# hamaadshah/gan_deeplearning4j

Hardware: AMD Instinct MI355X
Metric: images/sec (whole node) DCGAN 64x64 bf16 (higher is better)
Workload: dtype bf16; 1 GPU; model=dcgan64, global_batch=16384, z_size=128, parallelism=dp1

## Files before the change

gan_deeplearning4j_amd/ops/hip/gemm.hip:

```cpp

#include "conv_gather.h"

constexpr int TN_BM = 128, TN_BN = 128, TN_BK = 64;
constexpr int TN_TILE_B = TN_BM * TN_BK * 2;

DEV_INLINE bf16x8 tn_frag(const char* lds, int row, int kslot) {
  int byte = row * 128 + ((kslot ^ (row & 7)) * 16);
  return *(const bf16x8*)(lds + byte);
}

template <bool GATHER_A>
__global__ __launch_bounds__(256, 2) void gemm_tn_core(
    const unsigned short* __restrict__ A, const unsigned short* __restrict__ B,
    unsigned short* __restrict__ C, float* __restrict__ Cf,
    const float* __restrict__ bias, int M, int N, int K, long lda, long ldb,
    int act, float slope, ConvGather ga,
    const unsigned short* __restrict__ zp,
    float* __restrict__ bn_part) {
  __shared__ __attribute__((aligned(128))) char lds[4 * TN_TILE_B];
  auto abuf = [&](int i) -> char* { return lds + (i ? 2 * TN_TILE_B : 0); };
  auto bbuf = [&](int i) -> char* {
    return lds + TN_TILE_B + (i ? 2 * TN_TILE_B : 0);
  };

  const int nwgx = gridDim.x;
  const int bidx = xcd_remap(blockIdx.x, nwgx);
  const int m0 = bidx * TN_BM;
  const int n0 = blockIdx.y * TN_BN;

  const int wid = threadIdx.x >> 6;
  const int lane = threadIdx.x & 63;
  const int wr = wid >> 1, wc = wid & 1;
  const int fr = lane & 15, fq = lane >> 4;

  f32x4 acc[4][4];
  #pragma unroll
  for (int i = 0; i < 4; ++i)
    #pragma unroll
    for (int j = 0; j < 4; ++j) acc[i][j] = {0.f, 0.f, 0.f, 0.f};

  const int ntiles = K / TN_BK;
  TnGatherStager<256, unsigned short> gs;
  if (GATHER_A) {
    gs.init(ga, m0, M);
    gs.stage(A, ga, zp, 0, abuf(0));
  } else {
    tn_stage_rows<256, 4>(A, m0, M, lda, 0, abuf(0));
  }
  tn_stage_rows<256, 4>(B, n0, N, ldb, 0, bbuf(0));
  asm volatile("s_waitcnt vmcnt(0)" ::: "memory");
  __syncthreads();

  for (int t = 0; t < ntiles; ++t) {
    int cur = t & 1;
    if (t + 1 < ntiles) {
      if (GATHER_A)
        gs.stage(A, ga, zp, (t + 1) * TN_BK, abuf(cur ^ 1));
      else
        tn_stage_rows<256, 4>(A, m0, M, lda, (t + 1) * TN_BK, abuf(cur ^ 1));
      tn_stage_rows<256, 4>(B, n0, N, ldb, (t + 1) * TN_BK, bbuf(cur ^ 1));
    }
    const char* Al = abuf(cur);
    const char* Bl = bbuf(cur);
    #pragma unroll
    for (int kc = 0; kc < 2; ++kc) {
      bf16x8 a[4], b[4];
      #pragma unroll
      for (int mi = 0; mi < 4; ++mi)
        a[mi] = tn_frag(Al, wr * 64 + mi * 16 + fr, kc * 4 + fq);
      #pragma unroll
      for (int ni = 0; ni < 4; ++ni)
        b[ni] = tn_frag(Bl, wc * 64 + ni * 16 + fr, kc * 4 + fq);
      #pragma unroll
      for (int mi = 0; mi < 4; ++mi)
        #pragma unroll
        for (int ni = 0; ni < 4; ++ni)
          acc[mi][ni] = __builtin_amdgcn_mfma_f32_16x16x32_bf16(
              a[mi], b[ni], acc[mi][ni], 0, 0, 0);
    }
    asm volatile("s_waitcnt vmcnt(0)" ::: "memory");
    __syncthreads();
  }

  if (C != nullptr && (N & 7) == 0) {
    unsigned short* ctile = (unsigned short*)lds;
    __syncthreads();
    #pragma unroll
    for (int mi = 0; mi < 4; ++mi) {
      #pragma unroll
      for (int ni = 0; ni < 4; ++ni) {
        int lc = wc * 64 + ni * 16 + fr;
        float bv = bias != nullptr ? bias[min(n0 + lc, N - 1)] : 0.f;
        #pragma unroll
        for (int r = 0; r < 4; ++r) {
          int lr = wr * 64 + mi * 16 + fq * 4 + r;
          ctile[lr * 128 + lc] = f2bf(act_fwd(acc[mi][ni][r] + bv, act,
                                              slope));
        }
      }
    }
    __syncthreads();
    const int t = threadIdx.x;
    #pragma unroll
    for (int i = 0; i < 8; ++i) {
      int piece = i * 256 + t;
      int row = piece >> 4;
      int seg = piece & 15;
      int grow = m0 + row;
      int gcol = n0 + seg * 8;
      if (grow < M && gcol < N) {
        long crow = grow;
        if (GATHER_A && ga.mode == 2) crow = scatter_row(ga, grow);
        s16x8 v = *(const s16x8*)(ctile + row * 128 + seg * 8);
        if (gcol + 8 <= N) {
          *(s16x8*)(&C[crow * N + gcol]) = v;
        } else {
          for (int j = 0; j < 8 && gcol + j < N; ++j)
            C[crow * N + gcol + j] = (unsigned short)v[j];
        }
      }
    }
    if (bn_part != nullptr) {
      float* red = (float*)(lds + 2 * TN_TILE_B);
      const int col = t & 127;
      const int rl = t >> 7;
      float s = 0.f, ss = 0.f;
      for (int row = rl; row < 128; row += 2) {
        if (m0 + row < M) {
          float v = bf2f(ctile[row * 128 + col]);
          s += v;
          ss += v * v;
        }
      }
      red[t] = s;
      red[256 + t] = ss;
      __syncthreads();
      if (rl == 0 && n0 + col < N) {
        s += red[128 + col];
        ss += red[256 + 128 + col];
        bn_part[(long)blockIdx.x * 2 * N + n0 + col] = s;
        bn_part[(long)blockIdx.x * 2 * N + N + n0 + col] = ss;
      }
    }
    return;
  }
  #pragma unroll
  for (int mi = 0; mi < 4; ++mi) {
    #pragma unroll
    for (int ni = 0; ni < 4; ++ni) {
      int col = n0 + wc * 64 + ni * 16 + fr;
      if (col >= N) continue;
      float bv = bias != nullptr ? bias[col] : 0.f;
      #pragma unroll
      for (int r = 0; r < 4; ++r) {
        int row = m0 + wr * 64 + mi * 16 + fq * 4 + r;
        if (row >= M) continue;
        long crow = row;
        if (GATHER_A && ga.mode == 2) crow = scatter_row(ga, row);
        float v = act_fwd(acc[mi][ni][r] + bv, act, slope);
        if (C != nullptr)
          C[crow * N + col] = f2bf(v);
        else
          Cf[crow * N + col] = v;
      }
    }
  }
}

template <int KT, bool GATHER_A = false>
__global__ __launch_bounds__(256, 2) void gemm_tn_kshort(
    const unsigned short* __restrict__ A, const unsigned short* __restrict__ B,
    unsigned short* __restrict__ C, const float* __restrict__ bias, int M,
    int N, long lda, long ldb, int act, float slope, int direct_epi,
    ConvGather ga, const unsigned short* __restrict__ zp) {
  constexpr int NT = KT / TN_BK;
  __shared__ __attribute__((aligned(128))) char lds[2 * NT * TN_TILE_B];
  auto abuf = [&](int t) -> char* { return lds + t * TN_TILE_B; };
  auto bbuf = [&](int t) -> char* { return lds + (NT + t) * TN_TILE_B; };

  const int nwgx = gridDim.x;
  const int bidx = xcd_remap(blockIdx.x, nwgx);
  const int m0 = bidx * TN_BM;
  const int n0 = blockIdx.y * TN_BN;
  const int wid = threadIdx.x >> 6;
  const int lane = threadIdx.x & 63;
  const int wr = wid >> 1, wc = wid & 1;
  const int fr = lane & 15, fq = lane >> 4;

  f32x4 acc[4][4];
  #pragma unroll
  for (int i = 0; i < 4; ++i)
    #pragma unroll
    for (int j = 0; j < 4; ++j) acc[i][j] = {0.f, 0.f, 0.f, 0.f};

  TnGatherStager<256, unsigned short> gs;
  if (GATHER_A) gs.init(ga, m0, M);
  #pragma unroll
  for (int t = 0; t < NT; ++t) {
    if (GATHER_A)
      gs.stage(A, ga, zp, t * TN_BK, abuf(t));
    else
      tn_stage_rows<256, 4>(A, m0, M, lda, t * TN_BK, abuf(t));
    tn_stage_rows<256, 4>(B, n0, N, ldb, t * TN_BK, bbuf(t));
  }
  asm volatile("s_waitcnt vmcnt(0)" ::: "memory");
  __syncthreads();

  #pragma unroll
  for (int t = 0; t < NT; ++t) {
    const char* Al = abuf(t);
    const char* Bl = bbuf(t);
    #pragma unroll
    for (int kc = 0; kc < 2; ++kc) {
      bf16x8 a[4], b[4];
      #pragma unroll
      for (int mi = 0; mi < 4; ++mi)
        a[mi] = tn_frag(Al, wr * 64 + mi * 16 + fr, kc * 4 + fq);
      #pragma unroll
      for (int ni = 0; ni < 4; ++ni)
        b[ni] = tn_frag(Bl, wc * 64 + ni * 16 + fr, kc * 4 + fq);
      #pragma unroll
      for (int mi = 0; mi < 4; ++mi)
        #pragma unroll
        for (int ni = 0; ni < 4; ++ni)
          acc[mi][ni] = __builtin_amdgcn_mfma_f32_16x16x32_bf16(
              a[mi], b[ni], acc[mi][ni], 0, 0, 0);
    }
  }

  if ((N & 7) == 0 && direct_epi != 1) {
    unsigned short* ctile = (unsigned short*)lds;
    __syncthreads();
    #pragma unroll
    for (int mi = 0; mi < 4; ++mi) {
      #pragma unroll
      for (int ni = 0; ni < 4; ++ni) {
        int lc = wc * 64 + ni * 16 + fr;
        float bv = bias != nullptr ? bias[min(n0 + lc, N - 1)] : 0.f;
        #pragma unroll
        for (int r = 0; r < 4; ++r) {
          int lr = wr * 64 + mi * 16 + fq * 4 + r;
          ctile[lr * 128 + lc] = f2bf(act_fwd(acc[mi][ni][r] + bv, act,
                                              slope));
        }
      }
    }
    __syncthreads();
    const int t = threadIdx.x;
    #pragma unroll
    for (int i = 0; i < 8; ++i) {
      int piece = i * 256 + t;
      int row = piece >> 4;
      int seg = piece & 15;
      int grow = m0 + row;
      int gcol = n0 + seg * 8;
      if (grow < M && gcol + 8 <= N) {
        long crow = grow;
        if (GATHER_A && ga.mode == 2) crow = scatter_row(ga, grow);
        s16x8 v = *(const s16x8*)(ctile + row * 128 + seg * 8);
        if (direct_epi == 2)
          __builtin_nontemporal_store(v, (s16x8*)(&C[crow * N + gcol]));
        else
          *(s16x8*)(&C[crow * N + gcol]) = v;
      }
    }
    return;
  }
  #pragma unroll
  for (int mi = 0; mi < 4; ++mi)
    #pragma unroll
    for (int ni = 0; ni < 4; ++ni) {
      int col = n0 + wc * 64 + ni * 16 + fr;
      if (col >= N) continue;
      float bv = bias != nullptr ? bias[col] : 0.f;
      #pragma unroll
      for (int r = 0; r < 4; ++r) {
        int row = m0 + wr * 64 + mi * 16 + fq * 4 + r;
        if (row >= M) continue;
        long crow = row;
        if (GATHER_A && ga.mode == 2) crow = scatter_row(ga, row);
        C[crow * N + col] = f2bf(act_fwd(acc[mi][ni][r] + bv, act,
                                              slope));
      }
    }
}

constexpr int T2_BM = 256, T2_BN = 128, T2_BK = 64;
constexpr int T2_AT = T2_BM * T2_BK * 2;
constexpr int T2_BT = T2_BN * T2_BK * 2;

template <bool GATHER_A>
__global__ __launch_bounds__(512, 1) void gemm_tn_core256(
    const unsigned short* __restrict__ A, const unsigned short* __restrict__ B,
    unsigned short* __restrict__ C, const float* __restrict__ bias, int M,
    int N, int K, long lda, long ldb, int act, float slope, ConvGather ga,
    const unsigned short* __restrict__ zp) {
  extern __shared__ __attribute__((aligned(128))) char lds[];
  auto abuf = [&](int i) -> char* { return lds + (i ? T2_AT : 0); };
  auto bbuf = [&](int i) -> char* {
    return lds + 2 * T2_AT + (i ? T2_BT : 0);
  };

  const int nwgx = gridDim.x;
  const int bidx = xcd_remap(blockIdx.x, nwgx);
  const int m0 = bidx * T2_BM;
  const int n0 = blockIdx.y * T2_BN;

  const int wid = threadIdx.x >> 6;
  const int lane = threadIdx.x & 63;
  const int wr = wid >> 1, wc = wid & 1;
  const int fr = lane & 15, fq = lane >> 4;

  f32x4 acc[4][4];
  #pragma unroll
  for (int i = 0; i < 4; ++i)
    #pragma unroll
    for (int j = 0; j < 4; ++j) acc[i][j] = {0.f, 0.f, 0.f, 0.f};

  const int ntiles = K / T2_BK;
  TnGatherStager<512, unsigned short> gs;
  if (GATHER_A) {
    gs.init(ga, m0, M);
    gs.stage(A, ga, zp, 0, abuf(0));
  } else {
    tn_stage_rows<512, 4>(A, m0, M, lda, 0, abuf(0));
  }
  tn_stage_rows<512, 2>(B, n0, N, ldb, 0, bbuf(0));
  asm volatile("s_waitcnt vmcnt(0)" ::: "memory");
  __syncthreads();

  for (int t = 0; t < ntiles; ++t) {
    int cur = t & 1;
    if (t + 1 < ntiles) {
      if (GATHER_A)
        gs.stage(A, ga, zp, (t + 1) * T2_BK, abuf(cur ^ 1));
      else
        tn_stage_rows<512, 4>(A, m0, M, lda, (t + 1) * T2_BK, abuf(cur ^ 1));
      tn_stage_rows<512, 2>(B, n0, N, ldb, (t + 1) * T2_BK, bbuf(cur ^ 1));
    }
    const char* Al = abuf(cur);
    const char* Bl = bbuf(cur);
    #pragma unroll
    for (int kc = 0; kc < 2; ++kc) {
      bf16x8 a[4], b[4];
      #pragma unroll
      for (int mi = 0; mi < 4; ++mi)
        a[mi] = tn_frag(Al, wr * 64 + mi * 16 + fr, kc * 4 + fq);
      #pragma unroll
      for (int ni = 0; ni < 4; ++ni)
        b[ni] = tn_frag(Bl, wc * 64 + ni * 16 + fr, kc * 4 + fq);
      #pragma unroll
      for (int mi = 0; mi < 4; ++mi)
        #pragma unroll
        for (int ni = 0; ni < 4; ++ni)
          acc[mi][ni] = __builtin_amdgcn_mfma_f32_16x16x32_bf16(
              a[mi], b[ni], acc[mi][ni], 0, 0, 0);
    }
    asm volatile("s_waitcnt vmcnt(0)" ::: "memory");
    __syncthreads();
  }

  if ((N & 7) == 0) {
    unsigned short* ctile = (unsigned short*)lds;
    __syncthreads();
    #pragma unroll
    for (int mi = 0; mi < 4; ++mi) {
      #pragma unroll
      for (int ni = 0; ni < 4; ++ni) {
        int lc = wc * 64 + ni * 16 + fr;
        float bv = bias != nullptr ? bias[min(n0 + lc, N - 1)] : 0.f;
        #pragma unroll
        for (int r = 0; r < 4; ++r) {
          int lr = wr * 64 + mi * 16 + fq * 4 + r;
          ctile[lr * 128 + lc] = f2bf(act_fwd(acc[mi][ni][r] + bv, act,
                                              slope));
        }
      }
    }
    __syncthreads();
    const int t = threadIdx.x;
    #pragma unroll
    for (int i = 0; i < 8; ++i) {
      int piece = i * 512 + t;
      int row = piece >> 4;
      int seg = piece & 15;
      int grow = m0 + row;
      int gcol = n0 + seg * 8;
      if (grow < M && gcol < N) {
        s16x8 v = *(const s16x8*)(ctile + row * 128 + seg * 8);
        if (gcol + 8 <= N) {
          *(s16x8*)(&C[(long)grow * N + gcol]) = v;
        } else {
          for (int j = 0; j < 8 && gcol + j < N; ++j)
            C[(long)grow * N + gcol + j] = (unsigned short)v[j];
        }
      }
    }
    return;
  }
  #pragma unroll
  for (int mi = 0; mi < 4; ++mi) {
    #pragma unroll
    for (int ni = 0; ni < 4; ++ni) {
      int col = n0 + wc * 64 + ni * 16 + fr;
      if (col >= N) continue;
      float bv = bias != nullptr ? bias[col] : 0.f;
      #pragma unroll
      for (int r = 0; r < 4; ++r) {
        int row = m0 + wr * 64 + mi * 16 + fq * 4 + r;
        if (row >= M) continue;
        C[(long)row * N + col] = f2bf(act_fwd(acc[mi][ni][r] + bv, act,
                                              slope));
      }
    }
  }
}

constexpr int NT_BM = 128, NT_BN = 128, NT_BK = 64;
constexpr int NT_TILE_E = NT_BM * NT_BK;
constexpr int NT_THREADS = 512;

typedef __attribute__((ext_vector_type(4))) __bf16 bf16x4;

DEV_INLINE void nt_stage(const unsigned short* __restrict__ g, int k0, int K,
                         int c0, int L, long ldl,
                         const unsigned short* __restrict__ zp, char* lds) {
  const int t = threadIdx.x;
  const int wid = t >> 6;
  #pragma unroll
  for (int i = 0; i < 2; ++i) {
    int c = i * 512 + t;
    int w = c >> 3;
    int j = (c >> 1) & 3;
    int h = c & 1;
    int kb = w >> 3;
    int mb = w & 7;
    int row = k0 + kb * 4 + j;
    const unsigned short* src = zp;
    if (row < K) {
      int col = c0 + mb * 16 + h * 8;
      col = min(col, max(0, L - 8));
      src = g + (long)row * ldl + col;
    }
    char* dst = lds + (i * 512 + wid * 64) * 16;
    GLDS16(src, dst);
  }
}

struct NtGatherCols {
  int r[2], s[2], cc[2];
  bool in_rsc[2];

  DEV_INLINE void init(const ConvGather& g, int c0) {
    const int t = threadIdx.x;
    #pragma unroll
    for (int i = 0; i < 2; ++i) {
      int c = i * 512 + t;
      int w = c >> 3;
      int h = c & 1;
      int mb = w & 7;
      int kk = c0 + mb * 16 + h * 8;
      in_rsc[i] = kk < g.rsc;
      if (in_rsc[i])
        k_decode(g, (unsigned)kk, r[i], s[i], cc[i]);
      else
        r[i] = s[i] = cc[i] = 0;
    }
  }
};

DEV_INLINE void nt_stage_gather(const unsigned short* __restrict__ img,
                                const ConvGather& g, const NtGatherCols& gc,
                                int k0, int K,
                                const unsigned short* __restrict__ zp,
                                char* lds) {
  const int t = threadIdx.x;
  const int wid = t >> 6;
  #pragma unroll
  for (int i = 0; i < 2; ++i) {
    int c = i * 512 + t;
    int w = c >> 3;
    int j = (c >> 1) & 3;
    int kb = w >> 3;
    int np = k0 + kb * 4 + j;
    const unsigned short* src = zp;
    if (np < K && gc.in_rsc[i]) {
      int n, ho, wo;
      np_decode(g, (unsigned)np, n, ho, wo);
      bool valid;
      const unsigned short* p = gather_addr(g, img, n, ho, wo, gc.r[i],
                                            gc.s[i], gc.cc[i], valid);
      if (valid) src = p;
    }
    char* dst = lds + (i * 512 + wid * 64) * 16;
    GLDS16(src, dst);
  }
}

DEV_INLINE bf16x8 nt_tr_frag(const unsigned short* lds, int kc, int mb) {
  const int l = threadIdx.x & 63;
  const int g = l >> 4;
  int kb = kc * 8 + 2 * g;
  const unsigned short* a0 = lds + ((kb * 8 + mb) * 64 + (l & 15) * 4);
  bf16x4 lo = __builtin_amdgcn_ds_read_tr16_b64_v4bf16(
      (__attribute__((address_space(3))) bf16x4*)a0);
  bf16x4 hi = __builtin_amdgcn_ds_read_tr16_b64_v4bf16(
      (__attribute__((address_space(3))) bf16x4*)(a0 + 512));
  bf16x8 r;
  #pragma unroll
  for (int j = 0; j < 4; ++j) {
    r[j] = lo[j];
    r[4 + j] = hi[j];
  }
  return r;
}

template <int GMODE>
__global__ __launch_bounds__(NT_THREADS, 2) void gemm_nt_core(
    const unsigned short* __restrict__ A, const unsigned short* __restrict__ B,
    float* __restrict__ C, int M, int N, int K, long lda, long ldb,
    int kchunks_per_block, int use_atomic, ConvGather gg,
    const unsigned short* __restrict__ zp) {
  __shared__ __attribute__((aligned(128))) unsigned short lds[4 * NT_TILE_E];
  auto albuf = [&](int i) -> unsigned short* {
    return lds + (i ? 2 * NT_TILE_E : 0);
  };
  auto blbuf = [&](int i) -> unsigned short* {
    return lds + NT_TILE_E + (i ? 2 * NT_TILE_E : 0);
  };

  const int m0 = blockIdx.x * NT_BM;
  const int n0 = blockIdx.y * NT_BN;
  const int wid = threadIdx.x >> 6;
  const int lane = threadIdx.x & 63;
  const int wr = wid >> 2, wc = wid & 3;
  const int fr = lane & 15, fq = lane >> 4;

  f32x4 acc[4][2];
  #pragma unroll
  for (int i = 0; i < 4; ++i)
    #pragma unroll
    for (int j = 0; j < 2; ++j) acc[i][j] = {0.f, 0.f, 0.f, 0.f};

  const int kchunks = (K + NT_BK - 1) / NT_BK;
  int kt0 = blockIdx.z * kchunks_per_block;
  int kt1 = min(kt0 + kchunks_per_block, kchunks);
  if (kt0 >= kt1) return;

  NtGatherCols gca, gcb;
  if (GMODE == 1) gca.init(gg, m0);
  if (GMODE == 2) gcb.init(gg, n0);
  auto stage_a = [&](int kt, char* buf) {
    if (GMODE == 1)
      nt_stage_gather(A, gg, gca, kt * NT_BK, K, zp, buf);
    else
      nt_stage(A, kt * NT_BK, K, m0, M, lda, zp, buf);
  };
  auto stage_b = [&](int kt, char* buf) {
    if (GMODE == 2)
      nt_stage_gather(B, gg, gcb, kt * NT_BK, K, zp, buf);
    else
      nt_stage(B, kt * NT_BK, K, n0, N, ldb, zp, buf);
  };

  stage_a(kt0, (char*)albuf(0));
  stage_b(kt0, (char*)blbuf(0));
  asm volatile("s_waitcnt vmcnt(0)" ::: "memory");
  __syncthreads();

  for (int kt = kt0; kt < kt1; ++kt) {
    int cur = (kt - kt0) & 1;
    if (kt + 1 < kt1) {
      stage_a(kt + 1, (char*)albuf(cur ^ 1));
      stage_b(kt + 1, (char*)blbuf(cur ^ 1));
    }
    const unsigned short* Al = albuf(cur);
    const unsigned short* Bl = blbuf(cur);
    #pragma unroll
    for (int kc = 0; kc < 2; ++kc) {
      bf16x8 a[4], b[2];
      #pragma unroll
      for (int mi = 0; mi < 4; ++mi)
        a[mi] = nt_tr_frag(Al, kc, wr * 4 + mi);
      #pragma unroll
      for (int ni = 0; ni < 2; ++ni)
        b[ni] = nt_tr_frag(Bl, kc, wc * 2 + ni);
      #pragma unroll
      for (int mi = 0; mi < 4; ++mi)
        #pragma unroll
        for (int ni = 0; ni < 2; ++ni)
          acc[mi][ni] = __builtin_amdgcn_mfma_f32_16x16x32_bf16(
              a[mi], b[ni], acc[mi][ni], 0, 0, 0);
    }
    asm volatile("s_waitcnt vmcnt(0)" ::: "memory");
    __syncthreads();
  }

  #pragma unroll
  for (int mi = 0; mi < 4; ++mi) {
    #pragma unroll
    for (int ni = 0; ni < 2; ++ni) {
      int col = n0 + wc * 32 + ni * 16 + fr;
      if (col >= N) continue;
      #pragma unroll
      for (int r = 0; r < 4; ++r) {
        int row = m0 + wr * 64 + mi * 16 + fq * 4 + r;
        if (row >= M) continue;
        if (use_atomic)
          atomicAdd(&C[(long)row * N + col], acc[mi][ni][r]);
        else
          C[(long)row * N + col] = acc[mi][ni][r];
      }
    }
  }
}

template <bool GATHER_A>
static int launch_kshort(const void* A, const void* B, void* C,
                         const float* bias, int M, int N, int K, long lda,
                         long ldb, int act, float slope, int direct_epi,
                         const ConvGather& ga, const void* zp, hipStream_t s) {
  dim3 grid(ceil_div(M, TN_BM), ceil_div(N, TN_BN));
  auto* kern = K == 64 ? gemm_tn_kshort<64, GATHER_A>
                       : gemm_tn_kshort<128, GATHER_A>;
  hipLaunchKernelGGL(kern, grid, dim3(256), 0, s, (const unsigned short*)A,
                     (const unsigned short*)B, (unsigned short*)C, bias, M, N,
                     lda, ldb, act, slope, direct_epi, ga,
                     (const unsigned short*)zp);
  return (int)grid.x;
}

extern "C" {


static int t2_enabled() {
  static const int v = [] {
    int on = env_flag("GDLJ_TN256", 0);
    if (on) {
      (void)hipFuncSetAttribute(
          reinterpret_cast<const void*>(&gemm_tn_core256<false>),
          hipFuncAttributeMaxDynamicSharedMemorySize, 2 * T2_AT + 2 * T2_BT);
      (void)hipFuncSetAttribute(
          reinterpret_cast<const void*>(&gemm_tn_core256<true>),
          hipFuncAttributeMaxDynamicSharedMemorySize, 2 * T2_AT + 2 * T2_BT);
    }
    return on;
  }();
  return v;
}

static int kshort_enabled() {
  static const int v = env_flag("GDLJ_KSHORT", 1);
  return v;
}

int launch_gemm_tn(const void* A, const void* B, void* C_bf16, float* C_f32,
                   const float* bias, int M, int N, int K, long lda, long ldb,
                   int act, float slope, float* bn_part, hipStream_t s) {
  if (C_bf16 != nullptr && bn_part == nullptr && (K == 64 || K == 128) &&
      kshort_enabled()) {
    static const int depi = env_flag("GDLJ_KSHORT_EPI", 0);
    return launch_kshort<false>(A, B, C_bf16, bias, M, N, K, lda, ldb, act,
                                slope, depi, ConvGather{}, nullptr, s);
  }
  if (C_bf16 != nullptr && bn_part == nullptr &&
      gemm_tn_8p_eligible(M, N, K)) {
    ConvGather dummy{};
    return launch_gemm_tn_8p(A, B, C_bf16, bias, M, N, K, lda, ldb, act,
                             slope, 0, dummy, nullptr, s);
  }
  if (t2_enabled() && C_bf16 != nullptr && bn_part == nullptr &&
      M >= 8 * T2_BM) {
    dim3 grid(ceil_div(M, T2_BM), ceil_div(N, T2_BN));
    ConvGather dummy{};
    hipLaunchKernelGGL((gemm_tn_core256<false>), grid, dim3(512),
                       2 * T2_AT + 2 * T2_BT, s, (const unsigned short*)A,
                       (const unsigned short*)B, (unsigned short*)C_bf16,
                       bias, M, N, K, lda, ldb, act, slope, dummy, nullptr);
    return (int)grid.x;
  }
  dim3 grid(ceil_div(M, TN_BM), ceil_div(N, TN_BN));
  ConvGather dummy{};
  hipLaunchKernelGGL((gemm_tn_core<false>), grid, dim3(256), 0, s,
                     (const unsigned short*)A, (const unsigned short*)B,
                     (unsigned short*)C_bf16, C_f32, bias, M, N, K, lda, ldb,
                     act, slope, dummy, nullptr, bn_part);
  return (int)grid.x;
}

static int direct_conv_enabled() {
  static const int v = env_flag("GDLJ_DIRECT_CONV", 1);
  return v;
}

int launch_gemm_tn_gather(const void* img, const void* B, void* C_bf16,
                          const float* bias, int M, int N, int K, long ldb,
                          int act, float slope, ConvGather ga,
                          const void* zero_page, float* bn_part,
                          hipStream_t s) {
  if (bn_part == nullptr && ga.mode == 0 && ldb == K &&
      direct_conv_enabled() &&
      launch_conv_direct_smallc(img, B, C_bf16, bias, zero_page, ga.N, ga.H,
                                ga.W, ga.C, ga.Ho, ga.Wo, ga.R, ga.S,
                                ga.stride, ga.pad, N, K, act, slope, s))
    return ceil_div(M, 128);
  if (bn_part == nullptr && (K == 64 || K == 128) && kshort_enabled())
    return launch_kshort<true>(img, B, C_bf16, bias, M, N, K, 0, ldb, act,
                               slope, 0, ga, zero_page, s);
  if (bn_part == nullptr && gemm_tn_8p_eligible(M, N, K)) {
    return launch_gemm_tn_8p(img, B, C_bf16, bias, M, N, K, 0, ldb, act,
                             slope, 1, ga, zero_page, s);
  }
  if (t2_enabled() && bn_part == nullptr && ga.mode != 2 && M >= 8 * T2_BM) {
    dim3 grid(ceil_div(M, T2_BM), ceil_div(N, T2_BN));
    hipLaunchKernelGGL((gemm_tn_core256<true>), grid, dim3(512),
                       2 * T2_AT + 2 * T2_BT, s, (const unsigned short*)img,
                       (const unsigned short*)B, (unsigned short*)C_bf16,
                       bias, M, N, K, 0, ldb, act, slope, ga,
                       (const unsigned short*)zero_page);
    return (int)grid.x;
  }
  dim3 grid(ceil_div(M, TN_BM), ceil_div(N, TN_BN));
  hipLaunchKernelGGL((gemm_tn_core<true>), grid, dim3(256), 0, s,
                     (const unsigned short*)img, (const unsigned short*)B,
                     (unsigned short*)C_bf16, nullptr, bias, M, N, K, 0, ldb,
                     act, slope, ga, (const unsigned short*)zero_page,
                     bn_part);
  return (int)grid.x;
}

void launch_gemm_nt(const void* A, const void* B, float* C, int M, int N,
                    int K, long lda, long ldb, int splitk, int gmode,
                    ConvGather gg, const void* zp, hipStream_t s) {
  int kchunks = (K + NT_BK - 1) / NT_BK;
  if (splitk > kchunks) splitk = kchunks;
  int per_block = (kchunks + splitk - 1) / splitk;
  dim3 grid(ceil_div(M, NT_BM), ceil_div(N, NT_BN), splitk);
  int ua = splitk > 1 ? 1 : 0;
  const unsigned short* z = (const unsigned short*)zp;
  if (gmode == 1)
    hipLaunchKernelGGL((gemm_nt_core<1>), grid, dim3(NT_THREADS), 0, s,
                       (const unsigned short*)A, (const unsigned short*)B, C,
                       M, N, K, lda, ldb, per_block, ua, gg, z);
  else if (gmode == 2)
    hipLaunchKernelGGL((gemm_nt_core<2>), grid, dim3(NT_THREADS), 0, s,
                       (const unsigned short*)A, (const unsigned short*)B, C,
                       M, N, K, lda, ldb, per_block, ua, gg, z);
  else
    hipLaunchKernelGGL((gemm_nt_core<0>), grid, dim3(NT_THREADS), 0, s,
                       (const unsigned short*)A, (const unsigned short*)B, C,
                       M, N, K, lda, ldb, per_block, ua, gg, z);
}

}
```

gan_deeplearning4j_amd/ops/hip/launch_abi.h:

```cpp
#pragma once

#include <hip/hip_runtime.h>

constexpr int kPartRows = 2048;

struct FastDiv {
  unsigned long long mul;
  int shift;
  int d;
};

inline FastDiv make_fastdiv(int d) {
  int l = 0;
  while ((1 << l) < d) ++l;
  FastDiv f;
  f.shift = 32 + l;
  f.mul = ((1ULL << (32 + l)) + (unsigned long long)d - 1) /
          (unsigned long long)d;
  f.d = d;
  return f;
}

struct ConvGeom {
  int N, H, W, C;
  int Ho, Wo;
  int R, S;
  int stride, pad;
  int kpad;
};

struct PoolGeom {
  int N, H, W, C;
  int Ho, Wo;
  int k, stride;
};

struct ConvGather {
  int N, H, W, C;
  int Ho, Wo;
  int R, S, stride, pad;
  int rsc;
  int mode;
  int off_h, off_w;
  int oH, oW, oqh, oqw;
  FastDiv fC, fS, fWo, fHo, fStride;
};

inline ConvGather make_conv_gather(int N, int H, int W, int C, int Ho, int Wo,
                                   int R, int S, int stride, int pad,
                                   int mode = 0) {
  ConvGather g;
  g.N = N; g.H = H; g.W = W; g.C = C; g.Ho = Ho; g.Wo = Wo;
  g.R = R; g.S = S; g.stride = stride; g.pad = pad;
  g.rsc = R * S * C;
  g.mode = mode;
  g.off_h = g.off_w = 0;
  g.oH = g.oW = g.oqh = g.oqw = 0;
  g.fC = make_fastdiv(C);
  g.fS = make_fastdiv(S);
  g.fWo = make_fastdiv(Wo);
  g.fHo = make_fastdiv(Ho);
  g.fStride = make_fastdiv(stride);
  return g;
}

struct DgradDirectPlan {
  int kind;
  int bm;
  int qsplit;
  int lds_bytes;
};

struct DgradDirectArgs {
  const void* dy;
  const void* Wt;
  void* dx;
  const void* y0;
  float* part;
  const float* bias_fwd;
  float* stats_part;
  const void* zp;
  int Nb, H, W, C8, Ho, Wo, Ko8;
  long ldw;
  int R, S, pad, act;
  float slope;
};

extern "C" {

int launch_gemm_tn(const void* A, const void* B, void* C_bf16, float* C_f32,
                   const float* bias, int M, int N, int K, long lda, long ldb,
                   int act, float slope, float* bn_part, hipStream_t s);
int launch_gemm_tn_gather(const void* img, const void* B, void* C_bf16,
                          const float* bias, int M, int N, int K, long ldb,
                          int act, float slope, ConvGather ga,
                          const void* zero_page, float* bn_part,
                          hipStream_t s);
void launch_gemm_nt(const void* A, const void* B, float* C, int M, int N,
                    int K, long lda, long ldb, int splitk, int gmode,
                    ConvGather gg, const void* zp, hipStream_t s);

int gemm_tn_8p_eligible(int M, int N, int K);
int launch_gemm_tn_8p(const void* A, const void* B, void* C,
                      const float* bias, int M, int N, int K, long lda,
                      long ldb, int act, float slope, int gather,
                      ConvGather ga, const void* zp, hipStream_t s);
int launch_gemm_tn_8p_tweak(int tweak, const void* A, const void* B, void* C,
                            int M, int N, int K, long lda, long ldb,
                            hipStream_t s);

void launch_amax(const void* x, long n, unsigned* amax_bits, hipStream_t s);
void launch_fp8_make_scale(const unsigned* amax_bits, float* scale,
                           float* inv, hipStream_t s);
void launch_quant_fp8(const void* x, void* y, long n, const float* scale,
                      hipStream_t s);
void launch_quant_fp8_delayed(const void* x, void* y, long n,
                              const float* scale, unsigned* amax_bits,
                              hipStream_t s);
void launch_fp8_roll_scale(unsigned* amax_bits, float* scale, float* inv,
                           hipStream_t s);
void launch_gemm_tn_fp8(const void* A, const void* B, void* C,
                        const float* bias, const float* inv_qa,
                        const float* inv_qb, int M, int N, int K, long lda,
                        long ldb, int act, float slope, int gather,
                        ConvGather ga, const void* zp, hipStream_t s);

int gemm_tn_8p_fp8_eligible(int M, int N, int K);
int launch_gemm_tn_8p_fp8(const void* A, const void* B, void* C,
                          const float* bias, const float* inv_qa,
                          const float* inv_qb, int M, int N, int K, long lda,
                          long ldb, int act, float slope, int gather,
                          ConvGather ga, const void* zp, hipStream_t s);

int launch_conv_direct_smallc(const void* img, const void* Wp, void* C,
                              const float* bias, const void* zp, int Nb,
                              int H, int W, int C8, int Ho, int Wo, int R,
                              int S, int stride, int pad, int Kout, int kpad,
                              int act, float slope, hipStream_t s);

int conv_dgrad_direct_persist_enabled();
DgradDirectPlan conv_dgrad_direct_plan(int H, int W, int C8, int Ko8,
                                       long ldw, int R, int S, int stride,
                                       int pad, int allow_persist);
void launch_conv_dgrad_direct(const DgradDirectArgs& a, DgradDirectPlan plan,
                              hipStream_t s);

int launch_col2im_stats(const void* dcol, void* din, ConvGeom g,
                        const float* bias, int act, float slope, float* part,
                        hipStream_t s);
int launch_col2im_dact(const void* dcol, void* din, ConvGeom g,
                       const void* y0, int act, float slope, float* part,
                       hipStream_t s);
void launch_im2col(const void* in, void* col, ConvGeom g, hipStream_t s);
void launch_col2im(const void* dcol, void* din, ConvGeom g, const float* bias,
                   int act, float slope, hipStream_t s);

void launch_maxpool_fwd(const void* in, void* out, void* argmax, PoolGeom g,
                        hipStream_t s);
void launch_maxpool_bwd(const void* dout, const void* argmax, void* din,
                        PoolGeom g, hipStream_t s);
void launch_upsample_fwd(const void* in, void* out, int n, int h, int w,
                         int c, int scale, hipStream_t s);
void launch_upsample_bwd(const void* dout, void* din, int n, int h, int w,
                         int c, int scale, hipStream_t s);

void launch_act_fwd(const void* x, void* y, long n, int act, float slope,
                    hipStream_t s);
void launch_act_bwd(const void* dy, const void* y, void* dx, long n, int act,
                    float slope, hipStream_t s);
int launch_act_bwd_bias(const void* dy, const void* y, void* dx,
                        float* scratch, long m, int n, int act, float slope,
                        hipStream_t s);
int launch_col_sum_part(const void* a, float* scratch, long m, int n,
                        hipStream_t s);
void launch_col_sum_sum2(const float* scratch, int gx, int n, float* out,
                         hipStream_t s);
void launch_col_sum(const void* a, float* out, long m, int n, hipStream_t s);
void launch_bce_fwd(const void* logits, const void* labels, float* loss_sum,
                    long n, hipStream_t s);
void launch_bce_bwd(const void* logits, const void* labels, void* dlogits,
                    float gscale, long n, hipStream_t s);
void launch_softmax_xent_fwd(const void* logits, const void* onehot,
                             float* loss_sum, void* probs, int rows, int cols,
                             hipStream_t s);
void launch_softmax_xent_bwd(const void* probs, const void* onehot,
                             void* dlogits, float gscale, long n,
                             hipStream_t s);

int dropout_grid_cap();
int dropout_block_size();
void launch_dropout_fwd(const void* x, void* y, void* mask,
                        const void* state, long n, unsigned int thresh,
                        float scale, hipStream_t s);
void launch_dropout_bwd(const void* dy, const void* mask, void* dx, long n,
                        float scale, hipStream_t s);
void launch_gaussian_noise_fwd(const void* x, void* y, const void* state,
                               long n, float stddev, hipStream_t s);

void launch_bn_stats(const void* x, long m, int c, float* sum, float* sumsq,
                     hipStream_t s);
int launch_bn_stats_part(const void* x, long m, int c, float* scratch,
                         hipStream_t s);
void launch_bn_stats_sum2(const float* scratch, int gx, int c, float* sum,
                          float* sumsq, hipStream_t s);
void launch_bn_finalize(const float* sum, const float* sumsq, long m, int c,
                        float eps, float momentum, float* mean, float* istd,
                        float* running_mean, float* running_var,
                        hipStream_t s);
void launch_bn_apply(const void* x, void* y, long m, int c, const float* mean,
                     const float* istd, const float* gamma, const float* beta,
                     hipStream_t s);
void launch_bn_apply_eval(const void* x, void* y, long m, int c,
                          const float* rm, const float* rv, const float* gamma,
                          const float* beta, float eps, hipStream_t s);
void launch_bn_bwd_reduce(const void* x, const void* dy, long m, int c,
                          const float* mean, const float* istd, float* dgamma,
                          float* dbeta, hipStream_t s);
int launch_bn_bwd_reduce_part(const void* x, const void* dy, long m, int c,
                              const float* mean, const float* istd,
                              float* scratch, hipStream_t s);
void launch_bn_bwd_sum2(const float* scratch, int gx, int c, float* dgamma,
                        float* dbeta, hipStream_t s);
void launch_bn_bwd_apply(const void* x, const void* dy, void* dx, long m,
                         int c, const float* mean, const float* istd,
                         const float* gamma, const float* dgamma,
                         const float* dbeta, hipStream_t s);
int launch_bn_bwd_apply_act(const void* x, const void* dy, void* dx, long m,
                            int c, const float* mean, const float* istd,
                            const float* gamma, const float* dgamma,
                            const float* dbeta, int act, float slope,
                            float* bias_part, hipStream_t s);

void launch_fused_adam(void* param, const void* grad, float* master, float* m,
                       float* v, long n, int grad_is_bf16, int param_is_bf16,
                       float lr, float b1, float b2, float eps, float clip,
                       float l2, int t, const int* t_dev, hipStream_t s);
void launch_fused_rmsprop(void* param, const void* grad, float* master,
                          float* v, long n, int grad_is_bf16,
                          int param_is_bf16, float lr, float decay, float eps,
                          float clip, float l2, hipStream_t s);

}
```

Baseline: 161,400 images/s.

## Add 8-wave 256x256 NT GEMM kernel with transposed LDS reads for weight gradients

Adds a new NT GEMM kernel (used for large-K weight-gradient GEMMs) with 512 threads, 256x256 or 128x256 tiles, double-buffered LDS filled by direct global-to-LDS loads, ds_read_tr16 transposed fragment reads, and split-K sized to the CU count with XCD-aware block remapping. It dispatches ahead of the existing NT kernel when K is at least 32768 and M,N are at least 128. The aim is higher MFMA utilisation and more operand reuse in the long-K reductions. The trade-off is one block per CU, heavy register use, and fp32 atomics when split-K is active.

Measured after the change: 169,700 images/s (median of 6 runs). 5.1% higher.

```diff
diff --git a/gan_deeplearning4j_amd/ops/hip/gemm.hip b/gan_deeplearning4j_amd/ops/hip/gemm.hip
--- a/gan_deeplearning4j_amd/ops/hip/gemm.hip
+++ b/gan_deeplearning4j_amd/ops/hip/gemm.hip
@@ -732,6 +732,8 @@
 void launch_gemm_nt(const void* A, const void* B, float* C, int M, int N,
                     int K, long lda, long ldb, int splitk, int gmode,
                     ConvGather gg, const void* zp, hipStream_t s) {
+  if (launch_gemm_nt_8p(A, B, C, M, N, K, lda, ldb, splitk, gmode, gg, zp, s))
+    return;
   int kchunks = (K + NT_BK - 1) / NT_BK;
   if (splitk > kchunks) splitk = kchunks;
   int per_block = (kchunks + splitk - 1) / splitk;
diff --git a/gan_deeplearning4j_amd/ops/hip/gemm8p_nt.hip b/gan_deeplearning4j_amd/ops/hip/gemm8p_nt.hip
--- /dev/null
+++ b/gan_deeplearning4j_amd/ops/hip/gemm8p_nt.hip
@@ -0,0 +1,383 @@
+
+#include "conv_gather.h"
+
+namespace nt8 {
+
+constexpr int BK = 64;
+typedef __attribute__((ext_vector_type(4))) __bf16 bf16x4;
+
+template <int W>
+struct Op {
+  static constexpr int HALF_B = W * 64;
+  static constexpr int KBROW_B = W * 4;
+  static constexpr int TILE_B = W * 128;
+  static constexpr int NIT = W / 128;
+
+  static DEV_INLINE int kb_of(int i) {
+    const int wid = threadIdx.x >> 6;
+    const int lane = threadIdx.x & 63;
+    return W == 256 ? i * 8 + wid : wid * 2 + (lane >> 5);
+  }
+  static DEV_INLINE int colq() {
+    const int wid = threadIdx.x >> 6;
+    const int lane = threadIdx.x & 63;
+    int pw = W == 256 ? (lane >> 3) : ((lane >> 3) & 3);
+    int sw = W == 256 ? ((wid >> 1) & 1) : (wid & 1);
+    return ((pw ^ sw) << 4) + ((lane & 1) << 3);
+  }
+  static DEV_INLINE int rowq(int i) {
+    const int lane = threadIdx.x & 63;
+    return kb_of(i) * 4 + ((lane >> 1) & 3);
+  }
+  static DEV_INLINE int dstq(int i) {
+    const int wid = threadIdx.x >> 6;
+    return (W == 256 ? i * 8 + wid : wid) << 10;
+  }
+};
+
+template <int W>
+DEV_INLINE void stage_plain(const unsigned short* __restrict__ g, int k0,
+                            int K, int c0, int L, long ldl,
+                            const unsigned short* __restrict__ zp, int half,
+                            char* op) {
+  const int cq = c0 + half * (W / 2) + Op<W>::colq();
+  #pragma unroll
+  for (int i = 0; i < Op<W>::NIT; ++i) {
+    int row = k0 + Op<W>::rowq(i);
+    const unsigned short* src = zp;
+    if (row < K) {
+      int col = min(cq, max(0, L - 8));
+      src = g + (long)row * ldl + col;
+    }
+    GLDS16(src, op + half * Op<W>::HALF_B + Op<W>::dstq(i));
+  }
+}
+
+template <int W>
+struct GatherOp {
+  int r[2], s[2], cc[2];
+  bool in_rsc[2];
+  int n[Op<W>::NIT], ho[Op<W>::NIT], wo[Op<W>::NIT];
+
+  DEV_INLINE void init(const ConvGather& g, int c0) {
+    #pragma unroll
+    for (int h = 0; h < 2; ++h) {
+      int kk = c0 + h * (W / 2) + Op<W>::colq();
+      in_rsc[h] = kk < g.rsc;
+      if (in_rsc[h])
+        k_decode(g, (unsigned)kk, r[h], s[h], cc[h]);
+      else
+        r[h] = s[h] = cc[h] = 0;
+    }
+  }
+
+  DEV_INLINE void stage(const unsigned short* __restrict__ img,
+                        const ConvGather& g, int k0, int K,
+                        const unsigned short* __restrict__ zp, int half,
+                        char* op) {
+    #pragma unroll
+    for (int i = 0; i < Op<W>::NIT; ++i) {
+      int np = k0 + Op<W>::rowq(i);
+      if (half == 0) np_decode(g, (unsigned)np, n[i], ho[i], wo[i]);
+      const unsigned short* src = zp;
+      if (np < K && in_rsc[half]) {
+        bool valid;
+        const unsigned short* p = gather_addr(g, img, n[i], ho[i], wo[i],
+                                              r[half], s[half], cc[half],
+                                              valid);
+        if (valid) src = p;
+      }
+      GLDS16(src, op + half * Op<W>::HALF_B + Op<W>::dstq(i));
+    }
+  }
+};
+
+template <int W>
+DEV_INLINE bf16x8 tr_frag(const char* __restrict__ be,
+                          const char* __restrict__ bo, int half, int mbl,
+                          int kc) {
+  const char* p = ((mbl & 1) ? bo : be) + half * Op<W>::HALF_B +
+                  kc * 8 * Op<W>::KBROW_B + mbl * 128;
+  bf16x4 lo = __builtin_amdgcn_ds_read_tr16_b64_v4bf16(
+      (__attribute__((address_space(3))) bf16x4*)p);
+  bf16x4 hi = __builtin_amdgcn_ds_read_tr16_b64_v4bf16(
+      (__attribute__((address_space(3))) bf16x4*)(p + Op<W>::KBROW_B));
+  bf16x8 v;
+  #pragma unroll
+  for (int j = 0; j < 4; ++j) {
+    v[j] = lo[j];
+    v[4 + j] = hi[j];
+  }
+  return v;
+}
+
+}
+
+template <int GMODE, int BMT, int BNT>
+__global__ __launch_bounds__(512, 1) void gemm_nt_8p(
+    const unsigned short* __restrict__ A, const unsigned short* __restrict__ B,
+    float* __restrict__ C, int M, int N, int K, long lda, long ldb,
+    int kchunks_per_block, int use_atomic, int xcd, ConvGather gg,
+    const unsigned short* __restrict__ zp) {
+  using namespace nt8;
+  using OA = Op<BMT>;
+  using OB = Op<BNT>;
+  constexpr int BUF = OA::TILE_B + OB::TILE_B;
+  constexpr int MI = (BMT == 256 && BNT == 256) ? 8 : 4;
+  constexpr int MH = MI / 2;
+  constexpr int WCN = BNT / 64;
+  constexpr int INFL = OA::NIT + OB::NIT;
+  static_assert((BMT / (MI * 16)) * WCN == 8, "8 waves");
+  extern __shared__ __attribute__((aligned(16))) char lds[];
+
+  int bx = blockIdx.x, by = blockIdx.y, bz = blockIdx.z;
+  if (xcd) {
+    const int gx = gridDim.x, gy = gridDim.y;
+    const int nwg = gx * gy * (int)gridDim.z;
+    const int bid = xcd_remap(bx + gx * (by + gy * bz), nwg);
+    const int q = bid / gx;
+    bx = bid - q * gx;
+    bz = q / gy;
+    by = q - bz * gy;
+  }
+  const int m0 = bx * BMT;
+  const int n0 = by * BNT;
+
+  const int kchunks = (K + BK - 1) / BK;
+  const int kt0 = bz * kchunks_per_block;
+  const int kt1 = min(kt0 + kchunks_per_block, kchunks);
+  if (kt0 >= kt1) return;
+
+  if (__builtin_amdgcn_readfirstlane(threadIdx.x) >= 256)
+    __builtin_amdgcn_s_setprio(1);
+
+  const int wid = threadIdx.x >> 6;
+  const int lane = threadIdx.x & 63;
+  const int wr = wid / WCN, wc = wid % WCN;
+  const int fr = lane & 15, fq = lane >> 4;
+
+  f32x4 acc[MI][4];
+  #pragma unroll
+  for (int i = 0; i < MI; ++i)
+    #pragma unroll
+    for (int j = 0; j < 4; ++j) acc[i][j] = {0.f, 0.f, 0.f, 0.f};
+
+  auto abuf = [&](int tt) -> char* { return lds + (tt & 1) * BUF; };
+  auto bbuf = [&](int tt) -> char* { return abuf(tt) + OA::TILE_B; };
+
+  GatherOp<BMT> gca;
+  GatherOp<BNT> gcb;
+  if (GMODE == 1) gca.init(gg, m0);
+  if (GMODE == 2) gcb.init(gg, n0);
+  auto stage_a = [&](int tt, int half) {
+    int tc = min(tt, kt1 - 1);
+    if (GMODE == 1)
+      gca.stage(A, gg, tc * BK, K, zp, half, abuf(tc));
+    else
+      stage_plain<BMT>(A, tc * BK, K, m0, M, lda, zp, half, abuf(tc));
+  };
+  auto stage_b = [&](int tt, int half) {
+    int tc = min(tt, kt1 - 1);
+    if (GMODE == 2)
+      gcb.stage(B, gg, tc * BK, K, zp, half, bbuf(tc));
+    else
+      stage_plain<BNT>(B, tc * BK, K, n0, N, ldb, zp, half, bbuf(tc));
+  };
+
+#define NT8_VMWAIT()                                                         \
+  do {                                                                       \
+    if (INFL == 4)                                                           \
+      asm volatile("s_waitcnt vmcnt(4)" ::: "memory");                       \
+    else                                                                     \
+      asm volatile("s_waitcnt vmcnt(3)" ::: "memory");                       \
+  } while (0)
+
+  stage_a(kt0, 0);
+  stage_b(kt0, 0);
+  stage_a(kt0, 1);
+  stage_b(kt0, 1);
+  asm volatile("" ::: "memory");
+  stage_a(kt0 + 1, 0);
+  stage_b(kt0 + 1, 0);
+  NT8_VMWAIT();
+  __builtin_amdgcn_s_barrier();
+
+  const int sw = (fq & 1) * 128;
+  const int la = 2 * fq * OA::KBROW_B + fr * 8 + wr * MH * 128;
+  const int lb = 2 * fq * OB::KBROW_B + fr * 8 + wc * 2 * 128;
+
+  bf16x8 a[MH][2], blo[2][2], bhi[2][2];
+
+#define NT8_QUAD(MIH, NIH, BREG)                                             \
+  _Pragma("unroll") for (int kc = 0; kc < 2; ++kc)                           \
+      _Pragma("unroll") for (int mi = 0; mi < MH; ++mi)                      \
+      _Pragma("unroll") for (int ni = 0; ni < 2; ++ni)                       \
+      acc[(MIH)*MH + mi][(NIH)*2 + ni] =                                     \
+      __builtin_amdgcn_mfma_f32_16x16x32_bf16(                               \
+          a[mi][kc], BREG[ni][kc], acc[(MIH)*MH + mi][(NIH)*2 + ni], 0, 0,   \
+          0)
+
+#define NT8_BAR_MFMA(MIH, NIH, BREG)                                         \
+  __builtin_amdgcn_s_barrier();                                              \
+  asm volatile("s_waitcnt lgkmcnt(0)" ::: "memory");                         \
+  __builtin_amdgcn_sched_barrier(0);                                         \
+  NT8_QUAD(MIH, NIH, BREG);                                                  \
+  __builtin_amdgcn_s_barrier()
+
+  for (int t = kt0; t < kt1; ++t) {
+    const char* Ab = abuf(t);
+    const char* Bb = bbuf(t);
+    const char* ae = Ab + la + sw;
+    const char* ao = Ab + la - sw;
+    const char* be = Bb + lb + sw;
+    const char* bo = Bb + lb - sw;
+
+    #pragma unroll
+    for (int mi = 0; mi < MH; ++mi) {
+      a[mi][0] = tr_frag<BMT>(ae, ao, 0, mi, 0);
+      a[mi][1] = tr_frag<BMT>(ae, ao, 0, mi, 1);
+    }
+    #pragma unroll
+    for (int ni = 0; ni < 2; ++ni) {
+      blo[ni][0] = tr_frag<BNT>(be, bo, 0, ni, 0);
+      blo[ni][1] = tr_frag<BNT>(be, bo, 0, ni, 1);
+    }
+    stage_a(t + 1, 1);
+    NT8_BAR_MFMA(0, 0, blo);
+
+    #pragma unroll
+    for (int ni = 0; ni < 2; ++ni) {
+      bhi[ni][0] = tr_frag<BNT>(be, bo, 1, ni, 0);
+      bhi[ni][1] = tr_frag<BNT>(be, bo, 1, ni, 1);
+    }
+    stage_b(t + 1, 1);
+    NT8_BAR_MFMA(0, 1, bhi);
+
+    #pragma unroll
+    for (int mi = 0; mi < MH; ++mi) {
+      a[mi][0] = tr_frag<BMT>(ae, ao, 1, mi, 0);
+      a[mi][1] = tr_frag<BMT>(ae, ao, 1, mi, 1);
+    }
+    stage_a(t + 2, 0);
+    NT8_BAR_MFMA(1, 0, blo);
+
+    stage_b(t + 2, 0);
+    NT8_VMWAIT();
+    __builtin_amdgcn_s_barrier();
+    NT8_QUAD(1, 1, bhi);
+    __builtin_amdgcn_s_barrier();
+  }
+#undef NT8_BAR_MFMA
+#undef NT8_QUAD
+#undef NT8_VMWAIT
+
+  asm volatile("s_waitcnt vmcnt(0)" ::: "memory");
+
+  #pragma unroll
+  for (int mi = 0; mi < MI; ++mi) {
+    #pragma unroll
+    for (int ni = 0; ni < 4; ++ni) {
+      int col = n0 + (ni >> 1) * (BNT / 2) + (wc * 2 + (ni & 1)) * 16 + fr;
+      if (col >= N) continue;
+      #pragma unroll
+      for (int r = 0; r < 4; ++r) {
+        int row = m0 + (mi / MH) * (BMT / 2) + (wr * MH + mi % MH) * 16 +
+                  fq * 4 + r;
+        if (row >= M) continue;
+        if (use_atomic)
+          atomicAdd(&C[(long)row * N + col], acc[mi][ni][r]);
+        else
+          C[(long)row * N + col] = acc[mi][ni][r];
+      }
+    }
+  }
+}
+
+extern "C" {
+
+static int nt8_enabled() {
+  const char* e = getenv("GDLJ_NT8P");
+  return !(e != nullptr && e[0] == '0' && e[1] == '\0');
+}
+
+static int nt8_ncu() {
+  static const int v = [] {
+    int dev = 0, n = 0;
+    (void)hipGetDevice(&dev);
+    if (hipDeviceGetAttribute(&n, hipDeviceAttributeMultiprocessorCount,
+                              dev) != hipSuccess || n <= 0)
+      n = 256;
+    return n;
+  }();
+  return v;
+}
+
+static void nt8_set_attrs() {
+  static const int once = [] {
+    #define NT8_SETATTR(G, BM_, BN_)                                         \
+      (void)hipFuncSetAttribute(                                             \
+          reinterpret_cast<const void*>(&gemm_nt_8p<G, BM_, BN_>),           \
+          hipFuncAttributeMaxDynamicSharedMemorySize, 2 * (BM_ + BN_) * 128)
+    NT8_SETATTR(0, 256, 256);
+    NT8_SETATTR(1, 256, 256);
+    NT8_SETATTR(2, 256, 256);
+    NT8_SETATTR(0, 128, 256);
+    NT8_SETATTR(2, 128, 256);
+    NT8_SETATTR(0, 256, 128);
+    NT8_SETATTR(1, 256, 128);
+    #undef NT8_SETATTR
+    return 1;
+  }();
+  (void)once;
+}
+
+constexpr int kNt8MinK = 32768;
+
+int launch_gemm_nt_8p(const void* A, const void* B, float* C, int M, int N,
+                      int K, long lda, long ldb, int splitk, int gmode,
+                      ConvGather gg, const void* zp, hipStream_t s) {
+  if (!nt8_enabled()) return 0;
+  if (const char* e = getenv("GDLJ_NT8P_MINK")) {
+    if (K < atoi(e)) return 0;
+  } else if (K < kNt8MinK || M < 128 || N < 128) {
+    return 0;
+  }
+  int bmt = 256, bnt = 256;
+  if (M <= 128 && gmode != 1) bmt = 128;
+  else if (N <= 128 && gmode != 2) bnt = 128;
+  nt8_set_attrs();
+  const int kchunks = (K + nt8::BK - 1) / nt8::BK;
+  const int gm = ceil_div(M, bmt), gn = ceil_div(N, bnt);
+  int sk = 1;
+  if (splitk > 1) {
+    sk = nt8_ncu() / (gm * gn);
+    if (sk > kchunks) sk = kchunks;
+    if (sk < 1) sk = 1;
+  }
+  const int per_block = (kchunks + sk - 1) / sk;
+  const int ua = splitk > 1 ? 1 : 0;
+  dim3 grid(gm, gn, sk);
+  const int lds_b = 2 * (bmt + bnt) * 128;
+  const char* xe = getenv("GDLJ_NT8P_XCD");
+  const int xcd = !(xe != nullptr && xe[0] == '0' && xe[1] == '\0');
+  #define NT8_LAUNCH(G, BM_, BN_)                                            \
+    hipLaunchKernelGGL((gemm_nt_8p<G, BM_, BN_>), grid, dim3(512), lds_b, s, \
+                       (const unsigned short*)A, (const unsigned short*)B,   \
+                       C, M, N, K, lda, ldb, per_block, ua, xcd, gg,         \
+                       (const unsigned short*)zp)
+  if (bmt == 128) {
+    if (gmode == 2) NT8_LAUNCH(2, 128, 256);
+    else NT8_LAUNCH(0, 128, 256);
+  } else if (bnt == 128) {
+    if (gmode == 1) NT8_LAUNCH(1, 256, 128);
+    else NT8_LAUNCH(0, 256, 128);
+  } else {
+    if (gmode == 1) NT8_LAUNCH(1, 256, 256);
+    else if (gmode == 2) NT8_LAUNCH(2, 256, 256);
+    else NT8_LAUNCH(0, 256, 256);
+  }
+  #undef NT8_LAUNCH
+  return 1;
+}
+
+}
diff --git a/gan_deeplearning4j_amd/ops/hip/launch_abi.h b/gan_deeplearning4j_amd/ops/hip/launch_abi.h
--- a/gan_deeplearning4j_amd/ops/hip/launch_abi.h
+++ b/gan_deeplearning4j_amd/ops/hip/launch_abi.h
@@ -108,6 +108,10 @@
 int launch_gemm_tn_8p_tweak(int tweak, const void* A, const void* B, void* C,
                             int M, int N, int K, long lda, long ldb,
                             hipStream_t s);
+
+int launch_gemm_nt_8p(const void* A, const void* B, float* C, int M, int N,
+                      int K, long lda, long ldb, int splitk, int gmode,
+                      ConvGather gg, const void* zp, hipStream_t s);
 
 void launch_amax(const void* x, long n, unsigned* amax_bits, hipStream_t s);
 void launch_fp8_make_scale(const unsigned* amax_bits, float* scale,
```
